# HankKung/Auto-Dynamic-DeepLab

Measured on AMD Instinct MI355X. Metric: Cityscapes 1024x2048 images/sec fwd+bwd @ bs=2/GPU, higher is better.
Workload: dtype f32 storage and accumulation; k x k contractions as f16x3 split-fp16 MFMA products; 1 GPU; ADD F=20 searched_arch/autodeeplab/genotype C=2 all exits, 1024x2048 bs=2/GPU fwd+CE+bwd+SGD(nesterov); global_batch=2, parallelism=dp1, sync_bn=False, hip_graph=True, math=f16x3

## Files before the change

auto-dynamic-deeplab_amd/csrc/conv.h:

```cpp
#pragma once
#include "common.h"

enum ConvKind : int {
  CK_GENERIC = 0,
  CK_PARITY = 1,
  CK_STEM0 = 2,
  CK_PW = 3,
  CK_PWK = 4,
  CK_K1S = 5,
  CK_HALO = 6,
  CK_SPLIT = 7,
  CK_SPLIT_S2D = 8,
  CK_C3N = 9,
};
inline bool conv_kind_halo(int kind) { return kind >= CK_HALO; }

struct ConvChoice {
  int kind;
  int v[4];
  int gx, gy, launches;
  int rows;
  size_t lds;
  int key;
  struct Cls { long P; int ph, pw, MH, MW, ntaps, kill, gx, gx0, slab_row, pt, ct; int taplist[9]; } cls[4];
  int ncls;
  long P;
  int HT, spr, ntiles, nT; long wp_blk;
  int planes, bct, dil_odd, s2d, nchunks, pack_blocks;
  int64_t pack_floats;
};

int conv_choose_fwd(const addk_conv_args* a, int mode, int mask, ConvChoice& c);
int conv_choose_dgrad(const addk_conv_dgrad_args* a, int mode, int mask, ConvChoice& c);
bool pw_choose_fwd(const addk_conv_args* a, ConvChoice& c);
bool pw_choose_dgrad(const addk_conv_dgrad_args* a, ConvChoice& c);
bool c3_choose_fwd(const addk_conv_args* a, int mode, int mask, ConvChoice& c);
bool c3_choose_dgrad(const addk_conv_dgrad_args* a, int mode, int mask, ConvChoice& c);
int pw_run_fwd(const ConvChoice& c, const addk_conv_args* a, hipStream_t st);
int pw_run_dgrad(const ConvChoice& c, const addk_conv_dgrad_args* a, hipStream_t st);
int c3_run_fwd(const ConvChoice& c, const addk_conv_args* a, hipStream_t st);
int c3_run_dgrad(const ConvChoice& c, const addk_conv_dgrad_args* a, hipStream_t st);
```

auto-dynamic-deeplab_amd/csrc/pw.hip:

```cpp
#include <stdlib.h>
#include <type_traits>
#include "conv.h"

namespace {

enum { PW_FWD = 0, PW_DGRAD = 1 };

struct PwK {
  addk_src src;
  int K;
  int Cn;
  const float* w; int ldw; int w_off;
  float* y; int ldy;
  const float* bias;
  double* slab; int slab_ld;
  addk_src dst; int accumulate;
  int P; int ntiles16; int rows;
  int gx, gy;
  const void* gap0; int H, W; const void* gap1; int RH, RW; float* rs_y; int rs_ldy;
};

template <int CT, int KG, int MODE, bool RED32, bool RS = false>
__device__ __forceinline__ void pw_body(const PwK& p, double (*red)[CT * 16][2]) {
  const int t = threadIdx.x, lane = t & 63, wave = t >> 6;
  const int li = lane & 15, kq = lane >> 4;
  const int n0 = blockIdx.y * (CT * 16);

  float4 wf[CT][KG];
  auto load_panel = [&]() {
#pragma unroll
    for (int i = 0; i < CT; ++i)
#pragma unroll
      for (int g = 0; g < KG; ++g) {
        const int n = n0 + i * 16 + li, k = 16 * g + 4 * kq;
        const bool ok = n < p.Cn && k < p.K;
        float4 v;
        if (MODE == PW_FWD) {
          v = ld4(ok ? p.w + (long)n * p.ldw + p.w_off + k : p.w);
        } else {
          const gfloat* b = (const gfloat*)(ok ? p.w + (long)k * p.ldw + p.w_off + n : p.w);
          const long st = ok ? p.ldw : 0;
          v = make_float4(b[0], b[st], b[2 * st], b[3 * st]);
        }
        v.x = ok ? v.x : 0.f; v.y = ok ? v.y : 0.f; v.z = ok ? v.z : 0.f; v.w = ok ? v.w : 0.f;
        wf[i][g] = v;
      }
  };
  load_panel();
  const bool relu = p.src.relu != 0;
  const bool pro = relu || p.src.a != nullptr;
  float4 pa[KG], pb[KG];
#pragma unroll
  for (int g = 0; g < KG; ++g) {
    const int k = 16 * g + 4 * kq;
    pa[g] = make_float4(1.f, 1.f, 1.f, 1.f); pb[g] = zero4();
    if (p.src.a) {
      const bool ok = k < p.K;
      const float4 av = ld4(p.src.a + (ok ? k : 0)), bv = ld4(p.src.b + (ok ? k : 0));
      pa[g].x = ok ? av.x : 1.f; pa[g].y = ok ? av.y : 1.f; pa[g].z = ok ? av.z : 1.f; pa[g].w = ok ? av.w : 1.f;
      pb[g].x = ok ? bv.x : 0.f; pb[g].y = ok ? bv.y : 0.f; pb[g].z = ok ? bv.z : 0.f; pb[g].w = ok ? bv.w : 0.f;
    }
  }

  typedef typename std::conditional<RED32, float, double>::type red_t;
  red_t s1[CT][4], s2[CT][4];
#pragma unroll
  for (int i = 0; i < CT; ++i)
#pragma unroll
    for (int e = 0; e < 4; ++e) { s1[i][e] = 0; s2[i][e] = 0; }

  const int wstride = p.gx * 4;
  float4 xf[KG];
  const float rs_sh = RS ? (float)p.RH / (float)p.H : 0.f, rs_sw = RS ? (float)p.RW / (float)p.W : 0.f;
  auto load_tile = [&](int tile, float4 (&x)[KG]) {
    const int pp = tile * 16 + li;
    if (RS) {
      const int hw = p.H * p.W, pc = pp < p.P ? pp : 0;
      const int n = pc / hw, rem = pc - n * hw, oh = rem / p.W, ow = rem - oh * p.W;
      int h0, h1, w0, w1; float lh0, lh1, lw0, lw1;
      src_index(oh, rs_sh, p.RH, h0, h1, lh0, lh1);
      src_index(ow, rs_sw, p.RW, w0, w1, lw0, lw1);
      const float* b = p.src.x + (long)n * p.RH * p.RW * p.src.ld;
      const long o00 = ((long)h0 * p.RW + w0) * p.src.ld, o01 = ((long)h0 * p.RW + w1) * p.src.ld;
      const long o10 = ((long)h1 * p.RW + w0) * p.src.ld, o11 = ((long)h1 * p.RW + w1) * p.src.ld;
#pragma unroll
      for (int g = 0; g < KG; ++g) {
        const int k = 16 * g + 4 * kq;
        const bool ok = pp < p.P && k < p.K;
        const float* bk = ok ? b + k : p.src.x;
        const float4 v00 = ld4(bk + (ok ? o00 : 0)), v01 = ld4(bk + (ok ? o01 : 0)), v10 = ld4(bk + (ok ? o10 : 0)), v11 = ld4(bk + (ok ? o11 : 0));
        float4 v = lerp4(v00, v01, v10, v11, lh0, lh1, lw0, lw1);
        if (p.rs_y && ok && blockIdx.y == 0) st4(p.rs_y + (long)pp * p.rs_ldy + k, v);
        v.x = ok ? v.x : 0.f; v.y = ok ? v.y : 0.f; v.z = ok ? v.z : 0.f; v.w = ok ? v.w : 0.f;
        x[g] = v;
      }
      return;
    }
#pragma unroll
    for (int g = 0; g < KG; ++g) {
      const int k = 16 * g + 4 * kq;
      const bool ok = pp < p.P && k < p.K;
      float4 v = ld4(ok ? p.src.x + (long)pp * p.src.ld + k : p.src.x);
      v.x = ok ? v.x : 0.f; v.y = ok ? v.y : 0.f; v.z = ok ? v.z : 0.f; v.w = ok ? v.w : 0.f;
      x[g] = v;
    }
  };
  for (int tile = blockIdx.x * 4 + wave; tile < p.ntiles16; tile += wstride) {
    load_tile(tile, xf);
    const int pp = tile * 16 + li;
    const bool pin = pp < p.P;
    float4 dxp[CT], dop[CT];
    if (MODE == PW_DGRAD) {
#pragma unroll
      for (int i = 0; i < CT; ++i) {
        const int c = n0 + i * 16 + kq * 4;
        const int nrem = pin ? p.Cn - c : 0;
        dxp[i] = ld4g(p.dst.x + (pin ? (long)pp * p.dst.ld + c : 0), nrem, true);
        dop[i] = zero4();
        if (p.accumulate) dop[i] = ld4g(p.y + (pin ? (long)pp * p.ldy + c : 0), nrem, true);
      }
    }
    if (pro) {
#pragma unroll
      for (int g = 0; g < KG; ++g) {
        float4 v = xf[g];
        v.x = fmaf(pa[g].x, v.x, pb[g].x); v.y = fmaf(pa[g].y, v.y, pb[g].y); v.z = fmaf(pa[g].z, v.z, pb[g].z); v.w = fmaf(pa[g].w, v.w, pb[g].w);
        if (relu) { v.x = fmaxf(v.x, 0.f); v.y = fmaxf(v.y, 0.f); v.z = fmaxf(v.z, 0.f); v.w = fmaxf(v.w, 0.f); }
        const bool ok = pp < p.P && 16 * g + 4 * kq < p.K;
        v.x = ok ? v.x : 0.f; v.y = ok ? v.y : 0.f; v.z = ok ? v.z : 0.f; v.w = ok ? v.w : 0.f;
        xf[g] = v;
      }
    }
    f32x4 acc[CT];
#pragma unroll
    for (int i = 0; i < CT; ++i) acc[i] = (f32x4){0.f, 0.f, 0.f, 0.f};
#pragma unroll
    for (int g = 0; g < KG; ++g) {
#pragma unroll
      for (int e = 0; e < 4; ++e)
#pragma unroll
        for (int i = 0; i < CT; ++i)
          acc[i] = __builtin_amdgcn_mfma_f32_16x16x4f32(get4(wf[i][g], e), get4(xf[g], e), acc[i], 0, 0, 0);
    }
    if (pin) {
#pragma unroll
      for (int i = 0; i < CT; ++i) {
        const int c = n0 + i * 16 + kq * 4;
        const int nrem = p.Cn - c;
        if (nrem <= 0) continue;
        float4 v = make_float4(acc[i][0], acc[i][1], acc[i][2], acc[i][3]);
        if (MODE == PW_FWD) {
          if (p.bias) { float4 b = ld4g(p.bias + c, nrem, false); v.x += b.x; v.y += b.y; v.z += b.z; v.w += b.w; }
          st4g(p.y + (long)pp * p.ldy + c, v, nrem, true);
          if (p.slab) {
#pragma unroll
            for (int e = 0; e < 4; ++e) { const red_t f = e < nrem ? (red_t)get4(v, e) : (red_t)0; s1[i][e] += f; s2[i][e] += f * f; }
          }
        } else {
          const float4 x = dxp[i];
          float4 av = make_float4(1.f, 1.f, 1.f, 1.f), bv = zero4();
          if (p.dst.a) { av = ld4g(p.dst.a + c, nrem, true); bv = ld4g(p.dst.b + c, nrem, true); }
          float4 g4;
#pragma unroll
          for (int e = 0; e < 4; ++e) {
            const float xe = get4(x, e), ae = get4(av, e), be = get4(bv, e), dz = get4(v, e);
            const bool m = (e < nrem) && (!p.dst.relu || fmaf(ae, xe, be) > 0.f);
            set4(g4, e, m ? dz * ae : 0.f);
            if (p.slab && m) { s1[i][e] += (red_t)dz * (red_t)xe; s2[i][e] += (red_t)dz; }
          }
          float* gp = p.y + (long)pp * p.ldy + c;
          if (p.accumulate) { const float4 o = dop[i]; g4.x += o.x; g4.y += o.y; g4.z += o.z; g4.w += o.w; }
          st4g(gp, g4, nrem, true);
        }
      }
    }
  }

  if (p.slab) {
#pragma unroll
    for (int i = 0; i < CT; ++i)
#pragma unroll
      for (int e = 0; e < 4; ++e) {
        red_t a = s1[i][e], b = s2[i][e];
#pragma unroll
        for (int m = 1; m < 16; m <<= 1) { a += __shfl_xor(a, m); b += __shfl_xor(b, m); }
        if (li == 0) { red[wave][i * 16 + kq * 4 + e][0] = (double)a; red[wave][i * 16 + kq * 4 + e][1] = (double)b; }
      }
    __syncthreads();
    if (t < CT * 16 && n0 + t < p.Cn) {
      gdouble* o = (gdouble*)p.slab + ((long)blockIdx.x * p.slab_ld + n0 + t) * 2;
      o[0] = red[0][t][0] + red[1][t][0] + red[2][t][0] + red[3][t][0];
      o[1] = red[0][t][1] + red[1][t][1] + red[2][t][1] + red[3][t][1];
      for (int r = blockIdx.x + p.gx; r < p.rows; r += p.gx) {
        gdouble* z = (gdouble*)p.slab + ((long)r * p.slab_ld + n0 + t) * 2;
        z[0] = 0.0; z[1] = 0.0;
      }
    }
  }
}

template <int CT, int KG, int MODE, bool RED32, bool RS = false>
__global__ void __launch_bounds__(256, (KG <= 3 && !RS && MODE == PW_FWD ? 4 : 3)) pw_kernel(const PwK p) {
  __shared__ double red[4][CT * 16][2];
  pw_body<CT, KG, MODE, RED32, RS>(p, red);
}
template <int CT, int KG, int MODE, bool RED32, bool RS = false>
__global__ void __launch_bounds__(256, (KG <= 3 && !RS && MODE == PW_FWD ? 4 : 3)) pw_batch_kernel(const PwK* __restrict__ tab) {
  __shared__ double red[4][CT * 16][2];
  const PwK p = tab[blockIdx.z];
  if ((int)blockIdx.x >= p.gx || (int)blockIdx.y >= p.gy) return;
  pw_body<CT, KG, MODE, RED32, RS>(p, red);
}

struct PwkK {
  addk_src src[ADDK_MAX_SRC]; int nsrc;
  int Cn; const float* w; int ldw; int w_off;
  float* y; int ldy; const float* bias;
  double* slab; int slab_ld;
  int P, ntiles16, rows, gx;
  int H, W; float* rs_y; int rs_ldy;
};

template <int CT, bool RED32, bool RS = false>
__global__ void __launch_bounds__(256, RS ? 2 : 3) pwk_kernel(const PwkK p) {
  __shared__ double red[4][CT * 16][2];
  const int t = threadIdx.x, lane = t & 63, wave = t >> 6, li = lane & 15, kq = lane >> 4;
  const int n0 = blockIdx.y * (CT * 16);
  typedef typename std::conditional<RED32, float, double>::type red_t;
  red_t s1[CT][4], s2[CT][4];
#pragma unroll
  for (int i = 0; i < CT; ++i)
#pragma unroll
    for (int e = 0; e < 4; ++e) { s1[i][e] = 0; s2[i][e] = 0; }
  bool nok[CT]; const float* wrow[CT];
#pragma unroll
  for (int i = 0; i < CT; ++i) {
    const int n = n0 + i * 16 + li;
    nok[i] = n < p.Cn;
    wrow[i] = p.w + (long)(nok[i] ? n : 0) * p.ldw + p.w_off;
  }
  const int wstride = p.gx * 4;
  for (int tile = blockIdx.x * 4 + wave; tile < p.ntiles16; tile += wstride) {
    const int pp = tile * 16 + li;
    const bool pok = pp < p.P;
    f32x4 acc[CT];
#pragma unroll
    for (int i = 0; i < CT; ++i) acc[i] = (f32x4){0.f, 0.f, 0.f, 0.f};
    struct Grp { float4 x, x01, x10, x11, a, b, w[CT]; float lh0, lh1, lw0, lw1; bool ok, pro, relu, rs, copy; int k; };
    int s = 0, g = 0, choff = 0;
    int rn = 0, roh = 0, row = 0;
    if (RS) {
      const int hw = p.H * p.W, pc = pok ? pp : 0;
      rn = pc / hw; const int rem = pc - rn * hw; roh = rem / p.W; row = rem - roh * p.W;
    }
    auto load = [&](Grp& G, int s_, int g_, int choff_) {
      const addk_src S = p.src[s_];
      const int k = 16 * g_ + 4 * kq;
      const bool kok = k < S.C;
      G.ok = kok && pok; G.pro = S.a != nullptr; G.relu = S.relu != 0;
      G.rs = RS && S.rs_hw != 0;
      if (G.rs) {
        const int RH = S.rs_hw >> 16, RW = S.rs_hw & 0xffff;
        int h0, h1, w0, w1;
        src_index(roh, (float)RH / (float)p.H, RH, h0, h1, G.lh0, G.lh1);
        src_index(row, (float)RW / (float)p.W, RW, w0, w1, G.lw0, G.lw1);
        const float* b = S.x + (G.ok ? (long)rn * RH * RW * S.ld + k : 0);
        G.x = ld4(b + (G.ok ? ((long)h0 * RW + w0) * S.ld : 0));
        G.x01 = ld4(b + (G.ok ? ((long)h0 * RW + w1) * S.ld : 0));
        G.x10 = ld4(b + (G.ok ? ((long)h1 * RW + w0) * S.ld : 0));
        G.x11 = ld4(b + (G.ok ? ((long)h1 * RW + w1) * S.ld : 0));
        G.copy = s_ == 0 && p.rs_y != nullptr && blockIdx.y == 0; G.k = k;
      } else
      G.x = ld4(S.x + (G.ok ? (long)pp * S.ld + k : 0));
      G.a = make_float4(1.f, 1.f, 1.f, 1.f); G.b = zero4();
      if (S.a) { G.a = ld4(S.a + (kok ? k : 0)); G.b = ld4(S.b + (kok ? k : 0)); }
#pragma unroll
      for (int i = 0; i < CT; ++i) G.w[i] = ld4(wrow[i] + (kok ? choff_ + k : 0));
    };
    auto advance = [&](int& s_, int& g_, int& choff_) {
      ++g_;
      if (16 * g_ >= p.src[s_].C) { choff_ += p.src[s_].C; g_ = 0; ++s_; }
    };
    auto compute = [&](const Grp& G) {
      float4 v = G.x;
      if (RS && G.rs) {
        v = lerp4(G.x, G.x01, G.x10, G.x11, G.lh0, G.lh1, G.lw0, G.lw1);
        if (G.copy && G.ok) st4(p.rs_y + (long)pp * p.rs_ldy + G.k, v);
      }
      v.x = fmaf(G.a.x, v.x, G.b.x); v.y = fmaf(G.a.y, v.y, G.b.y); v.z = fmaf(G.a.z, v.z, G.b.z); v.w = fmaf(G.a.w, v.w, G.b.w);
      if (G.relu) { v.x = fmaxf(v.x, 0.f); v.y = fmaxf(v.y, 0.f); v.z = fmaxf(v.z, 0.f); v.w = fmaxf(v.w, 0.f); }
      v.x = G.ok ? v.x : 0.f; v.y = G.ok ? v.y : 0.f; v.z = G.ok ? v.z : 0.f; v.w = G.ok ? v.w : 0.f;
#pragma unroll
      for (int e = 0; e < 4; ++e)
#pragma unroll
        for (int i = 0; i < CT; ++i) {
          acc[i] = __builtin_amdgcn_mfma_f32_16x16x4f32(get4(G.w[i], e), get4(v, e), acc[i], 0, 0, 0);
        }
    };
    Grp A, B;
    load(A, s, g, choff);
    while (true) {
      int s2_ = s, g2 = g, c2 = choff;
      advance(s2_, g2, c2);
      const bool more = s2_ < p.nsrc;
      if (more) load(B, s2_, g2, c2);
      compute(A);
      if (!more) break;
      s = s2_; g = g2; choff = c2;
      int s3 = s, g3 = g, c3 = choff;
      advance(s3, g3, c3);
      const bool more2 = s3 < p.nsrc;
      if (more2) load(A, s3, g3, c3);
      compute(B);
      if (!more2) break;
      s = s3; g = g3; choff = c3;
    }
    if (pok) {
#pragma unroll
      for (int i = 0; i < CT; ++i) {
        const int c = n0 + i * 16 + kq * 4;
        const int nrem = p.Cn - c;
        if (nrem <= 0) continue;
        float4 v = make_float4(acc[i][0], acc[i][1], acc[i][2], acc[i][3]);
        if (p.bias) { float4 b = ld4g(p.bias + c, nrem, false); v.x += b.x; v.y += b.y; v.z += b.z; v.w += b.w; }
        st4g(p.y + (long)pp * p.ldy + c, v, nrem, true);
        if (p.slab) {
#pragma unroll
          for (int e = 0; e < 4; ++e) { const red_t f = e < nrem ? (red_t)get4(v, e) : (red_t)0; s1[i][e] += f; s2[i][e] += f * f; }
        }
      }
    }
  }
  if (p.slab) {
#pragma unroll
    for (int i = 0; i < CT; ++i)
#pragma unroll
      for (int e = 0; e < 4; ++e) {
        red_t a = s1[i][e], b = s2[i][e];
#pragma unroll
        for (int m = 1; m < 16; m <<= 1) { a += __shfl_xor(a, m); b += __shfl_xor(b, m); }
        if (li == 0) { red[wave][i * 16 + kq * 4 + e][0] = (double)a; red[wave][i * 16 + kq * 4 + e][1] = (double)b; }
      }
    __syncthreads();
    if (t < CT * 16 && n0 + t < p.Cn) {
      gdouble* o = (gdouble*)p.slab + ((long)blockIdx.x * p.slab_ld + n0 + t) * 2;
      o[0] = red[0][t][0] + red[1][t][0] + red[2][t][0] + red[3][t][0];
      o[1] = red[0][t][1] + red[1][t][1] + red[2][t][1] + red[3][t][1];
      for (int r = blockIdx.x + p.gx; r < p.rows; r += p.gx) {
        gdouble* z = (gdouble*)p.slab + ((long)r * p.slab_ld + n0 + t) * 2;
        z[0] = 0.0; z[1] = 0.0;
      }
    }
  }
}

struct PwCfg { int ct, kg, red32, gx, gy, rs; };
static bool pw_config(PwK& k, int rows, PwCfg& c) {
  c.rs = k.RH != 0;
  c.kg = cdiv(k.K, 16);
  if (!(c.kg == 3 || c.kg == 5)) return false;
  c.ct = c.kg == 5 ? 2 : 3;
  if (cdiv(k.Cn, 16) < c.ct) c.ct = cdiv(k.Cn, 16);
  if (c.ct < 1) c.ct = 1;
  k.rows = rows;
  c.gx = rows;
  const int tpw = 2;
  if (c.gx > cdiv(k.ntiles16, 4 * tpw)) c.gx = cdiv(k.ntiles16, 4 * tpw);
  if (c.gx < 1) c.gx = 1;
  c.gy = cdiv(k.Cn, 16 * c.ct);
  c.red32 = k.P >= 4096;
  k.gx = c.gx; k.gy = c.gy;
  return true;
}

template <int CT, int KG, int MODE, bool RED32, bool RS>
int pw_go(dim3 grid, hipStream_t st, const PwK* one, const PwK* tab) {
  if (tab) hipLaunchKernelGGL((pw_batch_kernel<CT, KG, MODE, RED32, RS>), grid, dim3(256), 0, st, tab);
  else hipLaunchKernelGGL((pw_kernel<CT, KG, MODE, RED32, RS>), grid, dim3(256), 0, st, *one);
  return addk_check_launch(tab ? "pw_conv_batch" : "pw_conv");
}
int pw_dispatch(const PwCfg& c, int mode, dim3 grid, hipStream_t st, const PwK* one, const PwK* tab) {
#define ADDK_PW_GO(CT_, KG_, MODE_, RS_) \
  (c.red32 ? pw_go<CT_, KG_, MODE_, true, RS_>(grid, st, one, tab) : pw_go<CT_, KG_, MODE_, false, RS_>(grid, st, one, tab))
#define ADDK_PW(CT_, KG_) \
  if (c.ct == CT_ && c.kg == KG_) { \
    if (mode == PW_DGRAD) return ADDK_PW_GO(CT_, KG_, PW_DGRAD, false); \
    return c.rs ? ADDK_PW_GO(CT_, KG_, PW_FWD, true) : ADDK_PW_GO(CT_, KG_, PW_FWD, false); }
  ADDK_PW(1, 3) ADDK_PW(2, 3) ADDK_PW(3, 3)
  ADDK_PW(1, 5) ADDK_PW(2, 5)
#undef ADDK_PW
#undef ADDK_PW_GO
  addk_set_error(tab ? "pw_batch: no instantiation" : "pw_conv: no instantiation");
  return ADDK_ERR_UNSUPPORTED;
}

template <int CT, bool RED32, bool RS>
int pwk_go(dim3 grid, hipStream_t st, const PwkK& k) {
  hipLaunchKernelGGL((pwk_kernel<CT, RED32, RS>), grid, dim3(256), 0, st, k);
  return addk_check_launch("pwk_conv");
}
int pwk_dispatch(int ct, int rs, int red32, dim3 grid, hipStream_t st, const PwkK& k) {
#define ADDK_PWK(CT_) \
  if (ct == CT_) { \
    if (rs) return red32 ? pwk_go<CT_, true, true>(grid, st, k) : pwk_go<CT_, false, true>(grid, st, k); \
    return red32 ? pwk_go<CT_, true, false>(grid, st, k) : pwk_go<CT_, false, false>(grid, st, k); }
  ADDK_PWK(1) ADDK_PWK(2) ADDK_PWK(3)
#undef ADDK_PWK
  addk_set_error("pwk_conv: no instantiation");
  return ADDK_ERR_UNSUPPORTED;
}

template <typename K>
void fwd_slab_pixels(const addk_conv_args* a, K& k) {
  k.slab = (double*)a->stats; k.slab_ld = a->stats_ld > 0 ? a->stats_ld : a->Cout;
  k.P = a->N * a->OH * a->OW; k.ntiles16 = cdiv(k.P, 16);
}

bool pw_fill_fwd(const addk_conv_args* a, PwK& k) {
  if (a->nsrc != 1 || a->KH != 1 || a->KW != 1 || a->stride != 1 || a->pad != 0 || a->bias_n) return false;
  const addk_src& s = a->src[0];
  const int kg = cdiv(s.C, 16);
  if (!(kg == 3 || kg == 5) || !src_vec_ok(s) || !aligned16(a->y) || a->ldy % 4 || a->Cout % 4 || a->H != a->OH || a->W != a->OW) return false;
  if (!aligned16(a->w) || a->ldw % 4 || a->w_choff % 4) return false;
  k = PwK{};
  k.src = s; k.K = s.C; k.Cn = a->Cout; k.w = a->w; k.ldw = a->ldw; k.w_off = a->w_choff;
  k.y = a->y; k.ldy = a->ldy; k.bias = a->bias;
  fwd_slab_pixels(a, k);
  k.H = a->OH; k.W = a->OW;
  if (s.rs_hw) {
    k.RH = s.rs_hw >> 16; k.RW = s.rs_hw & 0xffff;
    if (k.RH < 1 || k.RW < 1) return false;
    k.rs_y = a->rs_y; k.rs_ldy = a->rs_ldy;
    if (k.rs_y && (!aligned16(k.rs_y) || k.rs_ldy % 4 || k.rs_ldy < s.C)) return false;
  }
  return true;
}
bool pw_fill_dgrad(const addk_conv_dgrad_args* a, PwK& k) {
  if (a->KH != 1 || a->KW != 1 || a->stride != 1 || a->pad != 0 || a->H != a->OH || a->W != a->OW) return false;
  const int kg = cdiv(a->Cout, 16);
  addk_src dy{a->dy, nullptr, nullptr, a->lddy, a->Cout, 0, 0};
  if (!(kg == 3 || kg == 5) || !src_vec_ok(dy) || !src_vec_ok(a->dst) || !aligned16(a->g) || a->ldg % 4) return false;
  k = PwK{};
  k.src = dy; k.K = a->Cout; k.Cn = a->dst.C; k.w = a->w; k.ldw = a->ldw; k.w_off = a->w_choff;
  k.y = a->g; k.ldy = a->ldg; k.slab = (double*)a->dab; k.slab_ld = a->dst.C;
  k.dst = a->dst; k.accumulate = a->accumulate;
  k.P = a->N * a->H * a->W; k.ntiles16 = cdiv(k.P, 16);
  return true;
}
inline int pw_key(const PwCfg& c, int mode) { return (mode << 12) | (c.ct << 8) | (c.kg << 4) | (c.rs << 1) | c.red32; }
inline void pw_key_decode(int key, PwCfg& c, int& mode) {
  mode = key >> 12; c.ct = (key >> 8) & 15; c.kg = (key >> 4) & 15; c.rs = (key >> 1) & 1; c.red32 = key & 1;
}
void pw_choice(ConvChoice& c, const PwCfg& g, int mode) {
  c.kind = CK_PW; c.v[0] = g.ct; c.v[1] = g.kg; c.v[2] = g.rs; c.v[3] = g.red32; c.gx = g.gx; c.gy = g.gy; c.key = pw_key(g, mode);
}
void pw_desc(const ConvChoice& c, PwK& k) { k.rows = c.rows; k.gx = c.gx; k.gy = c.gy; }


struct StemK {
  const float* x; int ld; int N, H, W, OH, OW;
  const float* w; int ldw;
  float* y; int ldy;
  double* slab; int slab_ld;
  int P, ntiles16, rows, gx;
};
template <int CT, bool RED32>
__global__ void __launch_bounds__(256) stem0_kernel(const StemK p) {
  __shared__ double red[4][CT * 16][2];
  const int t = threadIdx.x, lane = t & 63, wave = t >> 6, li = lane & 15, kq = lane >> 4;
  float wf[CT][9];
#pragma unroll
  for (int i = 0; i < CT; ++i)
#pragma unroll
    for (int tap = 0; tap < 9; ++tap)
      wf[i][tap] = kq < 3 ? ((const gfloat*)p.w)[(long)(i * 16 + li) * p.ldw + tap * 3 + kq] : 0.f;
  typedef typename std::conditional<RED32, float, double>::type red_t;
  red_t s1[CT][4], s2[CT][4];
#pragma unroll
  for (int i = 0; i < CT; ++i)
#pragma unroll
    for (int e = 0; e < 4; ++e) { s1[i][e] = 0; s2[i][e] = 0; }
  const int ohw = p.OH * p.OW;
  const gfloat* xg = (const gfloat*)p.x;
  for (int tile = blockIdx.x * 4 + wave; tile < p.ntiles16; tile += p.gx * 4) {
    const int pp = tile * 16 + li;
    const bool pok = pp < p.P;
    const int n = pp / ohw, rem = pp - n * ohw, oh = rem / p.OW, ow = rem - oh * p.OW;
    float xv[9];
#pragma unroll
    for (int tap = 0; tap < 9; ++tap) {
      const int ih = 2 * oh - 1 + tap / 3, iw = 2 * ow - 1 + tap % 3;
      const bool ok = pok && kq < 3 && (unsigned)ih < (unsigned)p.H && (unsigned)iw < (unsigned)p.W;
      const float v = xg[ok ? ((long)(n * p.H + ih) * p.W + iw) * p.ld + kq : 0];
      xv[tap] = ok ? v : 0.f;
    }
    f32x4 acc[CT];
#pragma unroll
    for (int i = 0; i < CT; ++i) acc[i] = (f32x4){0.f, 0.f, 0.f, 0.f};
#pragma unroll
    for (int tap = 0; tap < 9; ++tap)
#pragma unroll
      for (int i = 0; i < CT; ++i) acc[i] = __builtin_amdgcn_mfma_f32_16x16x4f32(wf[i][tap], xv[tap], acc[i], 0, 0, 0);
    if (pok) {
#pragma unroll
      for (int i = 0; i < CT; ++i) {
        const float4 v = make_float4(acc[i][0], acc[i][1], acc[i][2], acc[i][3]);
        st4(p.y + (long)pp * p.ldy + i * 16 + kq * 4, v);
        if (p.slab) {
#pragma unroll
          for (int e = 0; e < 4; ++e) { const red_t f = (red_t)get4(v, e); s1[i][e] += f; s2[i][e] += f * f; }
        }
      }
    }
  }
  if (p.slab) {
#pragma unroll
    for (int i = 0; i < CT; ++i)
#pragma unroll
      for (int e = 0; e < 4; ++e) {
        red_t a = s1[i][e], b = s2[i][e];
#pragma unroll
        for (int m = 1; m < 16; m <<= 1) { a += __shfl_xor(a, m); b += __shfl_xor(b, m); }
        if (li == 0) { red[wave][i * 16 + kq * 4 + e][0] = (double)a; red[wave][i * 16 + kq * 4 + e][1] = (double)b; }
      }
    __syncthreads();
    if (t < CT * 16) {
      gdouble* o = (gdouble*)p.slab + ((long)blockIdx.x * p.slab_ld + t) * 2;
      o[0] = red[0][t][0] + red[1][t][0] + red[2][t][0] + red[3][t][0];
      o[1] = red[0][t][1] + red[1][t][1] + red[2][t][1] + red[3][t][1];
      for (int r = blockIdx.x + p.gx; r < p.rows; r += p.gx) {
        gdouble* z = (gdouble*)p.slab + ((long)r * p.slab_ld + t) * 2;
        z[0] = 0.0; z[1] = 0.0;
      }
    }
  }
}

inline int gx_tiles16(long P, int rows) {
  int gx = rows;
  if (gx > cdiv(cdiv(P, 16), 4)) gx = cdiv(cdiv(P, 16), 4);
  return gx < 1 ? 1 : gx;
}
bool pwk_covers(const addk_conv_args* a, bool& rs) {
  rs = false;
  if (a->KH != 1 || a->KW != 1 || a->stride != 1 || a->pad != 0 || a->bias_n || a->H != a->OH || a->W != a->OW) return false;
  if (!aligned16(a->y) || a->ldy % 4 || a->Cout % 4 || !aligned16(a->w) || a->ldw % 4 || a->w_choff % 4) return false;
  int ktot = 0;
  for (int i = 0; i < a->nsrc; ++i) {
    if (!src_vec_ok(a->src[i])) return false;
    ktot += a->src[i].C;
    if (a->src[i].rs_hw) { rs = true; if ((a->src[i].rs_hw >> 16) < 1 || (a->src[i].rs_hw & 0xffff) < 1) return false; }
  }
  if (a->rs_y && (!a->src[0].rs_hw || !aligned16(a->rs_y) || a->rs_ldy % 4 || a->rs_ldy < a->src[0].C)) return false;
  if (ktot < 64 || a->Cout > 160 || (long)a->N * a->OH * a->OW < 1024) return false;
  return true;
}
bool stem0_covers(const addk_conv_args* a) {
  if (a->nsrc != 1 || a->KH != 3 || a->KW != 3 || a->stride != 2 || a->pad != 1 || a->dil != 1 || a->bias || a->bias_n) return false;
  const addk_src& s = a->src[0];
  if (s.C != 3 || s.ld < 3 || s.a || s.b || s.relu || a->Cout != 64 || a->cin_total != 3 || a->w_choff != 0) return false;
  if (!aligned16(a->y) || a->ldy % 4 || a->ldy < 64) return false;
  return a->OH == (a->H + 2 - 3) / 2 + 1 && a->OW == (a->W + 2 - 3) / 2 + 1;
}

struct K1sK {
  const float* dy; int lddy, K;
  const float* w; int ldw, w_off;
  addk_src dst; float* g; int ldg, accumulate;
  double* slab; int P, rows, gx, Cn;
};
template <int KMAX>
__global__ void __launch_bounds__(256) k1s_dgrad_kernel(const K1sK p) {
  __shared__ double red[4][256][2];
  const int t = threadIdx.x, lane = t & 63, wave = t >> 6;
  const int c = 4 * lane;
  const bool cok = c < p.Cn;
  float4 wq[KMAX];
#pragma unroll
  for (int k = 0; k < KMAX; ++k) wq[k] = (k < p.K && cok) ? ld4(p.w + (long)k * p.ldw + p.w_off + c) : zero4();
  float4 av = make_float4(1.f, 1.f, 1.f, 1.f), bv = zero4();
  if (p.dst.a && cok) { av = ld4(p.dst.a + c); bv = ld4(p.dst.b + c); }
  const bool relu = p.dst.relu != 0, acc = p.accumulate != 0;
  double s1[4] = {0.0, 0.0, 0.0, 0.0}, s2[4] = {0.0, 0.0, 0.0, 0.0};
  const gfloat* dyg = (const gfloat*)p.dy;
  auto finish = [&](int pp, const float4 dz, const float4 x, const float4 old) {
    float4 g4;
#pragma unroll
    for (int e = 0; e < 4; ++e) {
      const float xe = get4(x, e), ae = get4(av, e), be = get4(bv, e), d = get4(dz, e);
      const bool m = !relu || fmaf(ae, xe, be) > 0.f;
      set4(g4, e, m ? d * ae : 0.f);
      if (m) { s1[e] += (double)d * (double)xe; s2[e] += (double)d; }
    }
    if (acc) { g4.x += old.x; g4.y += old.y; g4.z += old.z; g4.w += old.w; }
    st4(p.g + (long)pp * p.ldg + c, g4);
  };
  const int nw = p.gx * 4;
  for (int p0 = blockIdx.x * 4 + wave; p0 < p.P; p0 += 2 * nw) {
    const int p1 = p0 + nw;
    const bool ok1 = p1 < p.P;
    const float d0 = lane < p.K ? dyg[(long)p0 * p.lddy + lane] : 0.f;
    const float d1 = (ok1 && lane < p.K) ? dyg[(long)p1 * p.lddy + lane] : 0.f;
    float4 x0 = zero4(), x1 = zero4(), o0 = zero4(), o1 = zero4();
    if (cok) {
      x0 = ld4(p.dst.x + (long)p0 * p.dst.ld + c);
      if (ok1) x1 = ld4(p.dst.x + (long)p1 * p.dst.ld + c);
      if (acc) { o0 = ld4(p.g + (long)p0 * p.ldg + c); if (ok1) o1 = ld4(p.g + (long)p1 * p.ldg + c); }
    }
    float4 a0 = zero4(), a1 = zero4();
#pragma unroll
    for (int k = 0; k < KMAX; ++k) {
      const float u0 = __int_as_float(__builtin_amdgcn_readlane(__float_as_int(d0), k)), u1 = __int_as_float(__builtin_amdgcn_readlane(__float_as_int(d1), k));
      a0.x = fmaf(u0, wq[k].x, a0.x); a0.y = fmaf(u0, wq[k].y, a0.y); a0.z = fmaf(u0, wq[k].z, a0.z); a0.w = fmaf(u0, wq[k].w, a0.w);
      a1.x = fmaf(u1, wq[k].x, a1.x); a1.y = fmaf(u1, wq[k].y, a1.y); a1.z = fmaf(u1, wq[k].z, a1.z); a1.w = fmaf(u1, wq[k].w, a1.w);
    }
    if (cok) { finish(p0, a0, x0, o0); if (ok1) finish(p1, a1, x1, o1); }
  }
  if (p.slab) {
#pragma unroll
    for (int e = 0; e < 4; ++e) { red[wave][c + e][0] = s1[e]; red[wave][c + e][1] = s2[e]; }
    __syncthreads();
    if (t < p.Cn) {
      gdouble* o = (gdouble*)p.slab + ((long)blockIdx.x * p.Cn + t) * 2;
      o[0] = red[0][t][0] + red[1][t][0] + red[2][t][0] + red[3][t][0];
      o[1] = red[0][t][1] + red[1][t][1] + red[2][t][1] + red[3][t][1];
      for (int r = blockIdx.x + p.gx; r < p.rows; r += p.gx) {
        gdouble* z = (gdouble*)p.slab + ((long)r * p.Cn + t) * 2;
        z[0] = 0.0; z[1] = 0.0;
      }
    }
  }
}
bool k1s_covers(const addk_conv_dgrad_args* a) {
  if (a->KH != 1 || a->KW != 1 || a->stride != 1 || a->pad != 0 || a->H != a->OH || a->W != a->OW) return false;
  if (a->Cout > 32 || a->dst.C < 128 || a->dst.C > 256 || a->dst.C % 4) return false;
  if (!src_vec_ok(a->dst) || !aligned16(a->g) || a->ldg % 4 || !aligned16(a->w) || a->ldw % 4 || a->w_choff % 4) return false;
  return !a->dst.a || (aligned16(a->dst.a) && aligned16(a->dst.b));
}
}

bool pw_choose_fwd(const addk_conv_args* a, ConvChoice& c) {
  const long P = (long)a->N * a->OH * a->OW;
  if (stem0_covers(a)) {
    c.kind = CK_STEM0; c.v[0] = 4; c.v[1] = P >= 4096; c.gx = gx_tiles16(P, c.rows); c.gy = 1;
    return true;
  }
  PwK k; PwCfg g;
  if (pw_fill_fwd(a, k) && pw_config(k, c.rows, g)) { pw_choice(c, g, PW_FWD); return true; }
  bool rs;
  if (!pwk_covers(a, rs)) return false;
  int ct = cdiv(a->Cout, 16); if (ct > 3) ct = 3;
  c.kind = CK_PWK; c.v[0] = ct; c.v[1] = rs; c.v[2] = P >= 4096; c.gx = gx_tiles16(P, c.rows); c.gy = cdiv(a->Cout, 16 * ct);
  return true;
}
bool pw_choose_dgrad(const addk_conv_dgrad_args* a, ConvChoice& c) {
  PwK k; PwCfg g;
  if (pw_fill_dgrad(a, k)) {
    if (!pw_config(k, c.rows, g)) return false;
    pw_choice(c, g, PW_DGRAD);
    return true;
  }
  if (!k1s_covers(a)) return false;
  const long P = (long)a->N * a->H * a->W;
  c.kind = CK_K1S; c.v[0] = a->Cout <= 20 ? 20 : 32; c.gx = c.rows > cdiv(P, 8) ? cdiv(P, 8) : c.rows; c.gy = 1;
  if (c.gx < 1) c.gx = 1;
  return true;
}

int pw_run_fwd(const ConvChoice& c, const addk_conv_args* a, hipStream_t st) {
  if (c.kind == CK_PW) {
    PwK k; PwCfg g; int mode;
    pw_fill_fwd(a, k); pw_desc(c, k); pw_key_decode(c.key, g, mode);
    return pw_dispatch(g, mode, dim3(c.gx, c.gy), st, &k, nullptr);
  }
  if (c.kind == CK_STEM0) {
    const addk_src& s = a->src[0];
    StemK k{};
    k.x = s.x; k.ld = s.ld; k.N = a->N; k.H = a->H; k.W = a->W; k.OH = a->OH; k.OW = a->OW;
    k.w = a->w; k.ldw = a->ldw; k.y = a->y; k.ldy = a->ldy;
    fwd_slab_pixels(a, k); k.rows = c.rows; k.gx = c.gx;
    if (c.v[1]) hipLaunchKernelGGL((stem0_kernel<4, true>), dim3(c.gx), dim3(256), 0, st, k);
    else hipLaunchKernelGGL((stem0_kernel<4, false>), dim3(c.gx), dim3(256), 0, st, k);
    return addk_check_launch("stem0");
  }
  PwkK k{};
  for (int i = 0; i < a->nsrc; ++i) k.src[i] = a->src[i];
  k.nsrc = a->nsrc; k.Cn = a->Cout; k.w = a->w; k.ldw = a->ldw; k.w_off = a->w_choff;
  k.y = a->y; k.ldy = a->ldy; k.bias = a->bias;
  fwd_slab_pixels(a, k); k.rows = c.rows;
  k.H = a->OH; k.W = a->OW; k.rs_y = a->rs_y; k.rs_ldy = a->rs_ldy;
  k.gx = c.gx;
  return pwk_dispatch(c.v[0], c.v[1], c.v[2], dim3(c.gx, c.gy), st, k);
}
int pw_run_dgrad(const ConvChoice& c, const addk_conv_dgrad_args* a, hipStream_t st) {
  if (c.kind == CK_PW) {
    PwK k; PwCfg g; int mode;
    pw_fill_dgrad(a, k); pw_desc(c, k); pw_key_decode(c.key, g, mode);
    return pw_dispatch(g, mode, dim3(c.gx, c.gy), st, &k, nullptr);
  }
  K1sK k{};
  k.dy = a->dy; k.lddy = a->lddy; k.K = a->Cout; k.w = a->w; k.ldw = a->ldw; k.w_off = a->w_choff;
  k.dst = a->dst; k.g = a->g; k.ldg = a->ldg; k.accumulate = a->accumulate; k.slab = a->dab;
  k.P = a->N * a->H * a->W; k.rows = c.rows; k.gx = c.gx; k.Cn = a->dst.C;
  if (c.v[0] == 20) hipLaunchKernelGGL((k1s_dgrad_kernel<20>), dim3(c.gx), dim3(256), 0, st, k);
  else hipLaunchKernelGGL((k1s_dgrad_kernel<32>), dim3(c.gx), dim3(256), 0, st, k);
  return addk_check_launch("conv_dgrad (1x1, few output channels)");
}

extern "C" int addk_conv_fwd_resample_ok(const addk_conv_args* a) {
  if (!a || a->nsrc < 1 || a->nsrc > ADDK_MAX_SRC) return 0;
  bool any = false;
  for (int i = 0; i < a->nsrc; ++i) any = any || a->src[i].rs_hw != 0;
  ConvChoice c;
  return any && conv_choose_fwd(a, addk_get_conv_precision(), addk_get_fast_paths(), c) == ADDK_OK && (c.kind == CK_PW || c.kind == CK_PWK);
}

extern "C" int addk_conv_fwd_batch_key(const addk_conv_args* a) {
  ConvChoice c;
  return conv_choose_fwd(a, addk_get_conv_precision(), addk_get_fast_paths(), c) == ADDK_OK && c.kind == CK_PW ? c.key : -1;
}
extern "C" int addk_conv_dgrad_batch_key(const addk_conv_dgrad_args* a) {
  ConvChoice c;
  return conv_choose_dgrad(a, addk_get_conv_precision(), addk_get_fast_paths(), c) == ADDK_OK && c.kind == CK_PW ? c.key : -1;
}
template <typename Args>
static int64_t pw_batch_prepare(const Args* a, int32_t n, void* host_blob, int64_t blob_bytes, int64_t* meta,
                                int (*choose)(const Args*, int, int, ConvChoice&), bool (*fill)(const Args*, PwK&)) {
  const int mode = addk_get_conv_precision(), mask = addk_get_fast_paths();
  return batch_prepare<PwK>("conv_batch_prepare", a, n, host_blob, blob_bytes, meta, [=](const Args* x, PwK& k, BatchItem& b) {
    ConvChoice c;
    if (choose(x, mode, mask, c) || c.kind != CK_PW) return false;
    fill(x, k); pw_desc(c, k); b = BatchItem{c.key, c.gx, c.gy, 0};
    return true;
  });
}
extern "C" int64_t addk_conv_fwd_batch_prepare(const addk_conv_args* a, int32_t n, void* host_blob, int64_t blob_bytes, int64_t* meta) {
  return pw_batch_prepare(a, n, host_blob, blob_bytes, meta, conv_choose_fwd, pw_fill_fwd);
}
extern "C" int64_t addk_conv_dgrad_batch_prepare(const addk_conv_dgrad_args* a, int32_t n, void* host_blob, int64_t blob_bytes, int64_t* meta) {
  return pw_batch_prepare(a, n, host_blob, blob_bytes, meta, conv_choose_dgrad, pw_fill_dgrad);
}
extern "C" int addk_conv_batch_run(const void* dev_blob, const int64_t* meta, void* stream) {
  ADDK_REQUIRE(dev_blob && meta && meta[1] > 0 && meta[2] > 0 && meta[3] > 0, "conv_batch_run: bad args");
  PwCfg g; int mode;
  pw_key_decode((int)meta[0], g, mode);
  return pw_dispatch(g, mode, dim3((unsigned)meta[2], (unsigned)meta[3], (unsigned)meta[1]), (hipStream_t)stream, nullptr, reinterpret_cast<const PwK*>(dev_blob));
}
```

Measured before the change: 73.17 images/sec.

## Add multi-tile, software-pipelined pwk 1x1 conv kernel with DPP row reductions

New measurement: 73.41 images/sec, median of 6. About the same (+0.3%).

```diff
diff --git a/auto-dynamic-deeplab_amd/csrc/conv.h b/auto-dynamic-deeplab_amd/csrc/conv.h
--- a/auto-dynamic-deeplab_amd/csrc/conv.h
+++ b/auto-dynamic-deeplab_amd/csrc/conv.h
@@ -22,6 +22,7 @@
   int rows;
   size_t lds;
   int key;
+  int depth;
   struct Cls { long P; int ph, pw, MH, MW, ntaps, kill, gx, gx0, slab_row, pt, ct; int taplist[9]; } cls[4];
   int ncls;
   long P;
diff --git a/auto-dynamic-deeplab_amd/csrc/pw.hip b/auto-dynamic-deeplab_amd/csrc/pw.hip
--- a/auto-dynamic-deeplab_amd/csrc/pw.hip
+++ b/auto-dynamic-deeplab_amd/csrc/pw.hip
@@ -221,9 +221,22 @@
   int H, W; float* rs_y; int rs_ldy;
 };
 
-template <int CT, bool RED32, bool RS = false>
-__global__ void __launch_bounds__(256, RS ? 2 : 3) pwk_kernel(const PwkK p) {
-  __shared__ double red[4][CT * 16][2];
+template <int CTL>
+__device__ __forceinline__ float dpp_add_f32(float v) {
+  return v + __int_as_float(__builtin_amdgcn_update_dpp(0, __float_as_int(v), CTL, 0xF, 0xF, true));
+}
+__device__ __forceinline__ float row_sum16(float v) {
+  v = dpp_add_f32<0xB1>(v); v = dpp_add_f32<0x4E>(v); v = dpp_add_f32<0x141>(v);
+  return dpp_add_f32<0x140>(v);
+}
+__device__ __forceinline__ double row_sum16(double v) {
+#pragma unroll
+  for (int m = 1; m < 16; m <<= 1) v += __shfl_xor(v, m);
+  return v;
+}
+
+template <int CT, bool RED32, bool RS>
+__device__ __forceinline__ void pwk_one(const PwkK& p, double (*red)[CT * 16][2]) {
   const int t = threadIdx.x, lane = t & 63, wave = t >> 6, li = lane & 15, kq = lane >> 4;
   const int n0 = blockIdx.y * (CT * 16);
   typedef typename std::conditional<RED32, float, double>::type red_t;
@@ -337,8 +350,7 @@
 #pragma unroll
       for (int e = 0; e < 4; ++e) {
         red_t a = s1[i][e], b = s2[i][e];
-#pragma unroll
-        for (int m = 1; m < 16; m <<= 1) { a += __shfl_xor(a, m); b += __shfl_xor(b, m); }
+        a = row_sum16(a); b = row_sum16(b);
         if (li == 0) { red[wave][i * 16 + kq * 4 + e][0] = (double)a; red[wave][i * 16 + kq * 4 + e][1] = (double)b; }
       }
     __syncthreads();
@@ -352,6 +364,194 @@
       }
     }
   }
+}
+
+template <int CT, bool RED32, bool RS, int T, int D>
+__device__ __forceinline__ void pwk_tiles(const PwkK& p, double (*red)[4][CT * 16][2]) {
+  constexpr int R = D + 1, NQ = RS ? 4 : 1;
+  auto v4 = [](const float4 q) { return (f32x4){q.x, q.y, q.z, q.w}; };
+  auto f4 = [](const f32x4 q) { return make_float4(q[0], q[1], q[2], q[3]); };
+  const int t = threadIdx.x, lane = t & 63, wave = t >> 6, li = lane & 15, kq = lane >> 4;
+  const int n0 = blockIdx.y * (CT * 16);
+  typedef typename std::conditional<RED32, float, double>::type red_t;
+  red_t s1[CT][4], s2[CT][4];
+  auto clear = [&]() __attribute__((always_inline)) {
+#pragma unroll
+    for (int i = 0; i < CT; ++i)
+#pragma unroll
+      for (int e = 0; e < 4; ++e) { s1[i][e] = 0; s2[i][e] = 0; }
+  };
+  auto reduce = [&](int j) __attribute__((always_inline)) {
+#pragma unroll
+    for (int i = 0; i < CT; ++i)
+#pragma unroll
+      for (int e = 0; e < 4; ++e) {
+        red_t a = s1[i][e], b = s2[i][e];
+        a = row_sum16(a); b = row_sum16(b);
+        if (li == 0) { red[j][wave][i * 16 + kq * 4 + e][0] = (double)a; red[j][wave][i * 16 + kq * 4 + e][1] = (double)b; }
+      }
+  };
+  clear();
+  const float* wrow[CT];
+#pragma unroll
+  for (int i = 0; i < CT; ++i) {
+    const int n = n0 + i * 16 + li;
+    wrow[i] = p.w + (long)(n < p.Cn ? n : 0) * p.ldw + p.w_off;
+  }
+  {
+    const int tile0 = blockIdx.x * (4 * T) + wave;
+    int pp[T]; bool pok[T];
+    int rn[T], roh[T], row[T];
+    f32x4 acc[T][CT];
+#pragma unroll
+    for (int j = 0; j < T; ++j) {
+      pp[j] = (tile0 + 4 * j) * 16 + li;
+      pok[j] = pp[j] < p.P;
+#pragma unroll
+      for (int i = 0; i < CT; ++i) acc[j][i] = (f32x4){0.f, 0.f, 0.f, 0.f};
+      rn[j] = 0; roh[j] = 0; row[j] = 0;
+      if (RS) {
+        const int hw = p.H * p.W, pc = pok[j] ? pp[j] : 0;
+        rn[j] = pc / hw; const int rem = pc - rn[j] * hw; roh[j] = rem / p.W; row[j] = rem - roh[j] * p.W;
+      }
+    }
+    if (tile0 < p.ntiles16) {
+      struct Slot { f32x4 x[T][NQ]; float4 a, b, w[CT]; bool kok, relu, rs, copy; int rs_hw; };
+      struct Walk { int s, g, choff; };
+      auto advance = [&](Walk& u) __attribute__((always_inline)) {
+        if (u.s < p.nsrc) {
+          ++u.g;
+          if (16 * u.g >= p.src[u.s].C) { u.choff += p.src[u.s].C; u.g = 0; ++u.s; }
+        }
+      };
+      auto load_x = [&](Slot& G, const Walk& u) __attribute__((always_inline)) {
+        const bool live = u.s < p.nsrc;
+        const addk_src S = p.src[live ? u.s : 0];
+        const int k = 16 * u.g + 4 * kq;
+        G.kok = live && k < S.C; G.relu = S.relu != 0;
+        G.rs = RS && S.rs_hw != 0; G.rs_hw = S.rs_hw;
+        G.copy = RS && u.s == 0 && p.rs_y != nullptr && blockIdx.y == 0;
+#pragma unroll
+        for (int j = 0; j < T; ++j) {
+          const bool ok = G.kok && pok[j];
+          f32x4 q[4];
+          if (G.rs) {
+            const int RH = S.rs_hw >> 16, RW = S.rs_hw & 0xffff;
+            int h0, h1, w0, w1; float lh0, lh1, lw0, lw1;
+            src_index(roh[j], (float)RH / (float)p.H, RH, h0, h1, lh0, lh1);
+            src_index(row[j], (float)RW / (float)p.W, RW, w0, w1, lw0, lw1);
+            const float* b = S.x + (ok ? (long)rn[j] * RH * RW * S.ld + k : 0);
+            q[0] = v4(ld4(b + (ok ? ((long)h0 * RW + w0) * S.ld : 0)));
+            q[1] = v4(ld4(b + (ok ? ((long)h0 * RW + w1) * S.ld : 0)));
+            q[2] = v4(ld4(b + (ok ? ((long)h1 * RW + w0) * S.ld : 0)));
+            q[3] = v4(ld4(b + (ok ? ((long)h1 * RW + w1) * S.ld : 0)));
+          } else {
+            q[0] = v4(ld4(S.x + (ok ? (long)pp[j] * S.ld + k : 0)));
+            q[1] = q[2] = q[3] = (f32x4){0.f, 0.f, 0.f, 0.f};
+          }
+#pragma unroll
+          for (int c = 0; c < NQ; ++c) G.x[j][c] = q[c];
+        }
+      };
+      auto load_w = [&](Slot& G, const Walk& u) __attribute__((always_inline)) {
+        const bool live = u.s < p.nsrc;
+        const addk_src S = p.src[live ? u.s : 0];
+        const int k = 16 * u.g + 4 * kq;
+        const bool kok = live && k < S.C;
+        G.a = make_float4(1.f, 1.f, 1.f, 1.f); G.b = zero4();
+        if (S.a) { G.a = ld4(S.a + (kok ? k : 0)); G.b = ld4(S.b + (kok ? k : 0)); }
+#pragma unroll
+        for (int i = 0; i < CT; ++i) G.w[i] = ld4(wrow[i] + (kok ? u.choff + k : 0));
+      };
+      auto compute = [&](const Slot& G, int g16) __attribute__((always_inline)) {
+#pragma unroll
+        for (int j = 0; j < T; ++j) {
+          const bool ok = G.kok && pok[j];
+          float4 v = f4(G.x[j][0]);
+          if (RS && G.rs) {
+            const int RH = G.rs_hw >> 16, RW = G.rs_hw & 0xffff;
+            int h0, h1, w0, w1; float lh0, lh1, lw0, lw1;
+            src_index(roh[j], (float)RH / (float)p.H, RH, h0, h1, lh0, lh1);
+            src_index(row[j], (float)RW / (float)p.W, RW, w0, w1, lw0, lw1);
+            v = lerp4(f4(G.x[j][0]), f4(G.x[j][NQ > 1 ? 1 : 0]), f4(G.x[j][NQ > 1 ? 2 : 0]), f4(G.x[j][NQ > 1 ? 3 : 0]), lh0, lh1, lw0, lw1);
+            if (G.copy && ok) st4(p.rs_y + (long)pp[j] * p.rs_ldy + g16 + 4 * kq, v);
+          }
+          v.x = fmaf(G.a.x, v.x, G.b.x); v.y = fmaf(G.a.y, v.y, G.b.y); v.z = fmaf(G.a.z, v.z, G.b.z); v.w = fmaf(G.a.w, v.w, G.b.w);
+          if (G.relu) { v.x = fmaxf(v.x, 0.f); v.y = fmaxf(v.y, 0.f); v.z = fmaxf(v.z, 0.f); v.w = fmaxf(v.w, 0.f); }
+          v.x = ok ? v.x : 0.f; v.y = ok ? v.y : 0.f; v.z = ok ? v.z : 0.f; v.w = ok ? v.w : 0.f;
+#pragma unroll
+          for (int e = 0; e < 4; ++e)
+#pragma unroll
+            for (int i = 0; i < CT; ++i) {
+              acc[j][i] = __builtin_amdgcn_mfma_f32_16x16x4f32(get4(G.w[i], e), get4(v, e), acc[j][i], 0, 0, 0);
+            }
+        }
+      };
+      Slot sl[R];
+      Walk uw{0, 0, 0}, ux{0, 0, 0};
+      load_w(sl[0], uw);
+#pragma unroll
+      for (int r = 0; r < D; ++r) { load_x(sl[r], ux); advance(ux); }
+      for (bool more = true; more;) {
+#pragma unroll
+        for (int r = 0; r < R; ++r) {
+          if (more) {
+            const int g16 = 16 * uw.g;
+            advance(uw);
+            load_w(sl[(r + 1) % R], uw);
+            if (D == 1) load_x(sl[(r + 1) % R], uw);
+            else { load_x(sl[(r + D) % R], ux); advance(ux); }
+            compute(sl[r], g16);
+            more = uw.s < p.nsrc;
+          }
+        }
+      }
+    }
+#pragma unroll
+    for (int j = 0; j < T; ++j) {
+      if (pok[j]) {
+#pragma unroll
+        for (int i = 0; i < CT; ++i) {
+          const int c = n0 + i * 16 + kq * 4;
+          const int nrem = p.Cn - c;
+          if (nrem <= 0) continue;
+          float4 v = make_float4(acc[j][i][0], acc[j][i][1], acc[j][i][2], acc[j][i][3]);
+          if (p.bias) { float4 b = ld4g(p.bias + c, nrem, false); v.x += b.x; v.y += b.y; v.z += b.z; v.w += b.w; }
+          st4g(p.y + (long)pp[j] * p.ldy + c, v, nrem, true);
+          if (p.slab) {
+#pragma unroll
+            for (int e = 0; e < 4; ++e) { const red_t f = e < nrem ? (red_t)get4(v, e) : (red_t)0; s1[i][e] += f; s2[i][e] += f * f; }
+          }
+        }
+      }
+      if (p.slab) { reduce(j); clear(); }
+    }
+  }
+  if (p.slab) {
+    __syncthreads();
+    if (t < CT * 16 && n0 + t < p.Cn) {
+#pragma unroll
+      for (int j = 0; j < T; ++j) {
+        const int v = blockIdx.x * T + j;
+        if (v < p.gx) {
+          gdouble* o = (gdouble*)p.slab + ((long)v * p.slab_ld + n0 + t) * 2;
+          o[0] = red[j][0][t][0] + red[j][1][t][0] + red[j][2][t][0] + red[j][3][t][0];
+          o[1] = red[j][0][t][1] + red[j][1][t][1] + red[j][2][t][1] + red[j][3][t][1];
+          for (int r = v + p.gx; r < p.rows; r += p.gx) {
+            gdouble* z = (gdouble*)p.slab + ((long)r * p.slab_ld + n0 + t) * 2;
+            z[0] = 0.0; z[1] = 0.0;
+          }
+        }
+      }
+    }
+  }
+}
+
+template <int CT, bool RED32, bool RS = false, int T = 1, int D = 1>
+__global__ void __launch_bounds__(256, RS || T >= 4 ? 2 : 3) pwk_kernel(const PwkK p) {
+  __shared__ double red[T][4][CT * 16][2];
+  if constexpr (T == 1 && D == 1) pwk_one<CT, RED32, RS>(p, red[0]);
+  else pwk_tiles<CT, RED32, RS, T, D>(p, red);
 }
 
 struct PwCfg { int ct, kg, red32, gx, gy, rs; };
@@ -394,18 +594,30 @@
   return ADDK_ERR_UNSUPPORTED;
 }
 
-template <int CT, bool RED32, bool RS>
+#ifdef ADDK_PWK_TRY_T
+#define ADDK_PWK_TRY_T_RS (ADDK_PWK_TRY_T > 2 ? 2 : ADDK_PWK_TRY_T)
+#define ADDK_PWK_FORMS \
+  ADDK_PWK_FORM(false, ADDK_PWK_TRY_T, ADDK_PWK_TRY_D) ADDK_PWK_FORM(true, ADDK_PWK_TRY_T_RS, ADDK_PWK_TRY_D) \
+  ADDK_PWK_FORM(false, 1, ADDK_PWK_TRY_D) ADDK_PWK_FORM(true, 1, ADDK_PWK_TRY_D)
+#else
+#define ADDK_PWK_FORMS ADDK_PWK_FORM(false, 2, 1) ADDK_PWK_FORM(false, 1, 2)
+#endif
+template <int CT, bool RED32, bool RS, int T, int D>
 int pwk_go(dim3 grid, hipStream_t st, const PwkK& k) {
-  hipLaunchKernelGGL((pwk_kernel<CT, RED32, RS>), grid, dim3(256), 0, st, k);
+  hipLaunchKernelGGL((pwk_kernel<CT, RED32, RS, T, D>), grid, dim3(256), 0, st, k);
   return addk_check_launch("pwk_conv");
 }
-int pwk_dispatch(int ct, int rs, int red32, dim3 grid, hipStream_t st, const PwkK& k) {
+int pwk_dispatch(int ct, int rs, int red32, int T, int D, dim3 grid, hipStream_t st, const PwkK& k) {
 #define ADDK_PWK(CT_) \
-  if (ct == CT_) { \
-    if (rs) return red32 ? pwk_go<CT_, true, true>(grid, st, k) : pwk_go<CT_, false, true>(grid, st, k); \
-    return red32 ? pwk_go<CT_, true, false>(grid, st, k) : pwk_go<CT_, false, false>(grid, st, k); }
+  if (ct == CT_ && T == 1 && D == 1) { \
+    if (rs) return red32 ? pwk_go<CT_, true, true, 1, 1>(grid, st, k) : pwk_go<CT_, false, true, 1, 1>(grid, st, k); \
+    return red32 ? pwk_go<CT_, true, false, 1, 1>(grid, st, k) : pwk_go<CT_, false, false, 1, 1>(grid, st, k); }
   ADDK_PWK(1) ADDK_PWK(2) ADDK_PWK(3)
 #undef ADDK_PWK
+#define ADDK_PWK_FORM(RS_, T_, D_) \
+  if (ct == 3 && red32 && (rs != 0) == RS_ && T == T_ && D == D_) return pwk_go<3, true, RS_, T_, D_>(grid, st, k);
+  ADDK_PWK_FORMS
+#undef ADDK_PWK_FORM
   addk_set_error("pwk_conv: no instantiation");
   return ADDK_ERR_UNSUPPORTED;
 }
@@ -541,6 +753,21 @@
   if (gx > cdiv(cdiv(P, 16), 4)) gx = cdiv(cdiv(P, 16), 4);
   return gx < 1 ? 1 : gx;
 }
+struct PwkForm { int T, D; };
+inline PwkForm pwk_pick(long P, int ktot, int cout, bool rs, int nsrc, int rows) {
+  const int nt = cdiv(P, 16);
+  const bool built = cout > 32 && P >= 4096;
+  const bool one_trip = nt <= 4 * gx_tiles16(P, rows);
+#ifdef ADDK_PWK_TRY_T
+  (void)ktot; (void)nsrc;
+  if (!built || !one_trip) return PwkForm{1, 1};
+  return PwkForm{nt >= 1024 ? (rs ? ADDK_PWK_TRY_T_RS : ADDK_PWK_TRY_T) : 1, ADDK_PWK_TRY_D};
+#else
+  if (!built || rs || !one_trip) return PwkForm{1, 1};
+  if (nt >= 2048) return PwkForm{2, 1};
+  return PwkForm{1, nsrc == 1 && ktot >= 400 ? 2 : 1};
+#endif
+}
 bool pwk_covers(const addk_conv_args* a, bool& rs) {
   rs = false;
   if (a->KH != 1 || a->KW != 1 || a->stride != 1 || a->pad != 0 || a->bias_n || a->H != a->OH || a->W != a->OW) return false;
@@ -650,7 +877,12 @@
   bool rs;
   if (!pwk_covers(a, rs)) return false;
   int ct = cdiv(a->Cout, 16); if (ct > 3) ct = 3;
-  c.kind = CK_PWK; c.v[0] = ct; c.v[1] = rs; c.v[2] = P >= 4096; c.gx = gx_tiles16(P, c.rows); c.gy = cdiv(a->Cout, 16 * ct);
+  int ktot = 0;
+  for (int i = 0; i < a->nsrc; ++i) ktot += a->src[i].C;
+  const PwkForm f = pwk_pick(P, ktot, a->Cout, rs, a->nsrc, c.rows);
+  int lg = 0; while ((1 << lg) < f.T) ++lg;
+  c.kind = CK_PWK; c.v[0] = ct; c.v[1] = rs; c.v[2] = P >= 4096; c.v[3] = lg; c.depth = f.D;
+  c.gx = cdiv(gx_tiles16(P, c.rows), f.T); c.gy = cdiv(a->Cout, 16 * ct);
   return true;
 }
 bool pw_choose_dgrad(const addk_conv_dgrad_args* a, ConvChoice& c) {
@@ -689,8 +921,8 @@
   k.y = a->y; k.ldy = a->ldy; k.bias = a->bias;
   fwd_slab_pixels(a, k); k.rows = c.rows;
   k.H = a->OH; k.W = a->OW; k.rs_y = a->rs_y; k.rs_ldy = a->rs_ldy;
-  k.gx = c.gx;
-  return pwk_dispatch(c.v[0], c.v[1], c.v[2], dim3(c.gx, c.gy), st, k);
+  k.gx = gx_tiles16(k.P, c.rows);
+  return pwk_dispatch(c.v[0], c.v[1], c.v[2], 1 << c.v[3], c.depth, dim3(c.gx, c.gy), st, k);
 }
 int pw_run_dgrad(const ConvChoice& c, const addk_conv_dgrad_args* a, hipStream_t st) {
   if (c.kind == CK_PW) {
```
